# speedinghzl/DSRG

Hardware: AMD Instinct MI355X
Metric: images/sec DSRG train step (VGG16 321x321, 21-class) (higher is better)
Workload: dtype bf16 backbone (fp32 master weights) + f32/f64 supervision path

## Files before the change

### dsrg_amd/csrc/conv_igemm.hip

```cpp
#include "common.h"
#include <algorithm>
#include <cstdlib>
#include <cstring>
#include <functional>
#include <map>
#include <mutex>
#include <queue>
#include <vector>

namespace dsrg {
namespace {
typedef __attribute__((ext_vector_type(8))) __bf16 bf16x8;
typedef __attribute__((ext_vector_type(2))) __bf16 bf16x2;
typedef __attribute__((ext_vector_type(2))) float f32x2;
typedef __attribute__((ext_vector_type(16))) float f32x16;
typedef __attribute__((ext_vector_type(4))) float f32x4;
typedef __attribute__((address_space(3))) void lds_void;

constexpr int kBM = 256, kBN = 256;
constexpr int kOutRow = 128 * 2 + 16;
constexpr int kOutWave = 64 * kOutRow;
constexpr uint32_t kOob = 0x80000000u;
constexpr int kRowTab = 8 * kOutWave;
constexpr int kRowTabBytes = kBM * 4;
// ... 354 lines not shown
            const uint4 v = *reinterpret_cast<const uint4 *>(O + p * kOutRow + ch * 16);
            if (m >= 0 && chv) *reinterpret_cast<uint4 *>(G.y + (size_t)m * a.Cout + nw + ch * 8) = v;
        }
        return;
    }
    uint4 mk[16];
    if (G.mask) {
#pragma unroll
        for (int it = 0; it < 16; it++) {
            const int m = row_pixel(wm * 64 + it * 4 + (lane >> 4));
            mk[it] = (m >= 0 && chv) ? *reinterpret_cast<const uint4 *>(G.mask + (size_t)m * a.Cout + nw + (lane & 15) * 8) : make_uint4(0, 0, 0, 0);
        }
    } else {
#pragma unroll
        for (int it = 0; it < 16; it++) mk[it] = make_uint4(0x3f803f80u, 0x3f803f80u, 0x3f803f80u, 0x3f803f80u);
    }
    float cs[8] = {0, 0, 0, 0, 0, 0, 0, 0};
#pragma unroll
    for (int it = 0; it < 16; it++) {
        const int p = it * 4 + (lane >> 4), ch = lane & 15;
        const int m = row_pixel(wm * 64 + p);
        const uint4 v = *reinterpret_cast<const uint4 *>(O + p * kOutRow + ch * 16);
        uint32_t w4[4] = {v.x, v.y, v.z, v.w};
        const uint32_t y4[4] = {mk[it].x, mk[it].y, mk[it].z, mk[it].w};
#pragma unroll
        for (int e = 0; e < 4; e++) {
            const uint32_t lo = (int16_t)(y4[e] & 0xffffu) > 0 ? 0x0000ffffu : 0u;
            const uint32_t hi = (int32_t)y4[e] >= 0x10000 ? 0xffff0000u : 0u;
            w4[e] &= lo | hi;
            cs[2 * e] += __uint_as_float(w4[e] << 16);
            cs[2 * e + 1] += __uint_as_float(w4[e] & 0xffff0000u);
        }
        if (m >= 0 && chv) *reinterpret_cast<uint4 *>(G.y + (size_t)m * a.Cout + nw + ch * 8) = make_uint4(w4[0], w4[1], w4[2], w4[3]);
    }
    if (G.colsum) {
#pragma unroll
        for (int e = 0; e < 8; e++) {
            cs[e] += __shfl_xor(cs[e], 16);
            cs[e] += __shfl_xor(cs[e], 32);
        }
        float *slab = reinterpret_cast<float *>(O);
        if (lane < 16) {
            *reinterpret_cast<float4 *>(slab + lane * 8) = make_float4(cs[0], cs[1], cs[2], cs[3]);
            *reinterpret_cast<float4 *>(slab + lane * 8 + 4) = make_float4(cs[4], cs[5], cs[6], cs[7]);
        }
        __syncthreads();
        if (wm == 0) {
            const float *s0 = reinterpret_cast<const float *>(ig_lds + (wn * 4 + 0) * kOutWave);
            const float *s1 = reinterpret_cast<const float *>(ig_lds + (wn * 4 + 1) * kOutWave);
            const float *s2 = reinterpret_cast<const float *>(ig_lds + (wn * 4 + 2) * kOutWave);
            const float *s3 = reinterpret_cast<const float *>(ig_lds + (wn * 4 + 3) * kOutWave);
            float *dst = G.colsum + (size_t)tm * a.Cout + nw;
            dst[lane] = (s0[lane] + s1[lane]) + (s2[lane] + s3[lane]);
            if (nw + lane + 64 < a.Cout) dst[lane + 64] = (s0[lane + 64] + s1[lane + 64]) + (s2[lane + 64] + s3[lane + 64]);
        }
    }
}


__global__ __launch_bounds__(512, 2) void conv_igemm_kernel_64x2(IgemmArgs a) { conv_igemm_body(a, (int)blockIdx.x, (int)gridDim.x); }

struct IgemmSkArgs {
    IgemmArgs base;
    float *ws;
    uint32_t *flags;
    int units, tiles_total;
};
constexpr int kSkParts = 4;
using f32x4v = decltype(__builtin_amdgcn_raw_buffer_load_b128(rsrc_t(), 0, 0, 0));

__global__ __launch_bounds__(512, 2) void conv_igemm_sk_kernel(IgemmSkArgs k) {
    using C = ICfg<64, 2>;
    const IgemmArgs &a = k.base;
    extern __shared__ __attribute__((aligned(16))) unsigned char ig_lds[];
    const int tid = threadIdx.x, lane = tid & 63;
    const int wv = __builtin_amdgcn_readfirstlane(tid >> 6);
    const int l15 = lane & 15, g4 = lane >> 4;
    const int wn = wv >> 2, wm = wv & 3;
    int unit;
    {
        const int total = (int)gridDim.x, id = (int)blockIdx.x;
        const int q = total >> 3, r = total & 7, xcd = id & 7, kk = id >> 3;
        unit = (xcd < r ? xcd * (q + 1) : r * (q + 1) + (xcd - r) * q) + kk;
    }
    const int taps = a.taps, Cin = a.Cin, W = a.W, H = a.H;
    const int ktot = taps * Cin;
    const int nsteps = (Cin >> 6) * taps;
    const long long total_steps = (long long)k.tiles_total * nsteps;
    auto unit_start = [&](int u) { return (long long)u * total_steps / k.units; };
    const long long g1 = unit_start(unit + 1);
    const IgemmFrag fr(lane);
    const rsrc_t rws = make_rsrc(k.ws, (size_t)k.units * 32 * 512 * 16);
    const float floor_ = a.relu ? 0.0f : -__builtin_inff();

    for (long long g = unit_start(unit); g < g1;) {
        const int tile = (int)(g / nsteps);
        const int sb = (int)(g - (long long)tile * nsteps);
        const int se = (int)min((long long)nsteps, sb + (g1 - g));
        int t = tile;
        const int grp = t / a.tiles_per_group;
        t -= grp * a.tiles_per_group;
        const int tm = t / a.tiles_n, tn = t - tm * a.tiles_n;
        const int m0 = tm * kBM, n0 = tn * kBN;
        const IgemmGroup G = a.g[grp];
        const rsrc_t rx = make_rsrc(G.x, (size_t)a.M * Cin * 2);
        const rsrc_t rw = make_rsrc(G.w, (size_t)a.Cout * ktot * 2);
        const bool active = n0 + wn * 128 < a.Cout;

        uint32_t pbase0, wbase0, pvalid01 = 0, pvalid23 = 0;
        {
            const int r0 = wv * 32 + lane / C::CPR;
            const int c0 = (lane % C::CPR) ^ C::swz(r0);
            pbase0 = (uint32_t)(m0 + r0) * (uint32_t)(Cin * 2) + (uint32_t)c0 * 16u;
            wbase0 = (uint32_t)(n0 + r0) * (uint32_t)(ktot * 2) + (uint32_t)c0 * 16u;
#pragma unroll
            for (int i = 0; i < C::IPW; i++) {
                const int m = m0 + r0 + i * C::RPI;
                uint32_t valid = 0;
                if (m < a.M) {
                    const int hw = H * W;
                    const int bimg = m / hw, rem = m - bimg * hw, y = rem / W, x = rem - y * W;
                    if (taps == 9) {
#pragma unroll
                        for (int tap = 0; tap < 9; tap++) {
                            const int yy = y + (tap / 3 - 1) * G.dil, xx = x + (tap % 3 - 1) * G.dil;
                            if (yy >= 0 && yy < H && xx >= 0 && xx < W) valid |= 1u << tap;
                        }
                    } else {
                        valid = 1u;
                    }
                }
                if (i < 2) pvalid01 |= valid << (16 * i); else pvalid23 |= valid << (16 * (i - 2));
            }
        }
        auto issue = [&](int stage, int s) {
            const int cc = s / taps, tap = s - cc * taps;
            int dy = 0, dx = 0;
            if (taps == 9) { dy = tap / 3 - 1; dx = tap - (tap / 3) * 3 - 1; }
            const int toff = (dy * G.dil * W + dx * G.dil) * Cin * 2 + cc * 128;
            unsigned char *P = ig_lds + stage * C::STAGE + wv * (32 * C::ROW);
            unsigned char *Wt = P + kBM * C::ROW;
#pragma unroll
            for (int i = 0; i < C::IPW; i++) {
                const uint32_t bits = (i < 2 ? pvalid01 : pvalid23) >> (16 * (i & 1) + tap);
                const uint32_t off = ((pbase0 + (uint32_t)(i * C::RPI * Cin * 2)) ^ ((i & 1) ? 64u : 0u)) + (uint32_t)toff;
                __builtin_amdgcn_raw_ptr_buffer_load_lds(rx, (lds_void *)(P + i * (C::RPI * C::ROW)), 16, (bits & 1u) ? off : kOob, 0, 0, 0);
            }
#pragma unroll
            for (int i = 0; i < C::IPW; i++)
                __builtin_amdgcn_raw_ptr_buffer_load_lds(rw, (lds_void *)(Wt + i * (C::RPI * C::ROW)), 16, (i & 1) ? wbase0 ^ 64u : wbase0,
                                                         (uint32_t)s * C::ROW + (uint32_t)(i * C::RPI * ktot * 2), 0, 0);
        };

        f32x4 acc[8][4];
#pragma unroll
        for (int i = 0; i < 8; i++)
#pragma unroll
            for (int j = 0; j < 4; j++)
#pragma unroll
                for (int r = 0; r < 4; r++) acc[i][j][r] = 0.0f;

        issue(0, sb);
        if (!active) {
            for (int s = sb; s < se; s++) {
                wait_vm_barrier<0>();
                if (s + 1 < se) issue(((s - sb) & 1) ^ 1, s + 1);
            }
        } else {
            for (int s = sb; s < se; s++) {
                const int stage = (s - sb) & 1;
                wait_vm_barrier<0>();
                const bool more = s + 1 < se, late = wv >= 4;
                if (more && !late) issue(stage ^ 1, s + 1);
                igemm_mma_step(ig_lds + stage * C::STAGE + wm * (64 * C::ROW), ig_lds + stage * C::STAGE + kBM * C::ROW + wn * (128 * C::ROW), fr, acc,
                               more && late, [&]() { issue(stage ^ 1, s + 1); });
            }
        }
        __syncthreads();

        if (sb != 0) {
            if (active) {
#pragma unroll
                for (int i = 0; i < 8; i++)
#pragma unroll
                    for (int j = 0; j < 4; j++) {
                        f32x4v v = {__float_as_uint(acc[i][j][0]), __float_as_uint(acc[i][j][1]), __float_as_uint(acc[i][j][2]), __float_as_uint(acc[i][j][3])};
                        __builtin_amdgcn_raw_buffer_store_b128(v, rws, (uint32_t)((i * 4 + j) * 512 + tid) * 16u,
                                                               (uint32_t)unit * (32u * 512u * 16u), 16);
                    }
            }
            asm volatile("s_waitcnt vmcnt(0)" ::: "memory");
            __syncthreads();
            if (tid == 0) __hip_atomic_store(k.flags + unit, 1u, __ATOMIC_RELAXED, __HIP_MEMORY_SCOPE_AGENT);
        } else {
            bool ok = true;
            int nparts = 0;
            if (se != nsteps) {
                const long long tile_end = (long long)(tile + 1) * nsteps;
                while (unit + 1 + nparts < k.units && unit_start(unit + 1 + nparts) < tile_end) nparts++;
                volatile int &sk_ok = *reinterpret_cast<volatile int *>(ig_lds);
                if (tid == 0) {
                    int good = nparts <= kSkParts ? 1 : 0;
                    for (int p = 0; p < nparts && good; p++) {
                        unsigned spins = 0;
                        while (__hip_atomic_load(k.flags + unit + 1 + p, __ATOMIC_RELAXED, __HIP_MEMORY_SCOPE_AGENT) != 1u) {
                            __builtin_amdgcn_s_sleep(8);
                            if (++spins > (1u << 24)) { good = 0; break; }
                        }
                    }
                    if (good) __builtin_amdgcn_fence(__ATOMIC_ACQUIRE, "agent");
                    else __hip_atomic_store(k.flags + k.units, 1u, __ATOMIC_RELAXED, __HIP_MEMORY_SCOPE_AGENT);
                    sk_ok = good;
                }
                __syncthreads();
                ok = sk_ok != 0;
                __syncthreads();
            }
            if (active) {
                const float poison = ok ? 0.0f : __builtin_nanf("");
                unsigned char *O = ig_lds + wv * kOutWave;
                const int nw = n0 + wn * 128;
                const rsrc_t rb = make_rsrc(G.bias, G.bias ? (size_t)a.Cout * 4 : 0);
                const uint32_t seed_g = a.seed_lo + (uint32_t)grp * 0x9E3779B9u;
                f32x4v shares[2][kSkParts];
                float bq[2][4];
                auto fetch = [&](int gi, f32x4v (&dst)[kSkParts], float (&bias4)[4]) {
                    const int i = gi >> 2;
                    const uint32_t off = (uint32_t)(gi * 512 + tid) * 16u;
#pragma unroll
                    for (int p = 0; p < kSkParts; p++)
                        dst[p] = __builtin_amdgcn_raw_buffer_load_b128(rws, p < nparts ? off : kOob, (uint32_t)(unit + 1 + p) * (32u * 512u * 16u), 0);
#pragma unroll
                    for (int e = 0; e < 4; e++) bias4[e] = ld_f32(rb, (uint32_t)(nw + i * 16 + g4 * 4 + e) * 4u);
                };
                fetch(0, shares[0], bq[0]);
#pragma unroll
                for (int gi = 0; gi < 32; gi++) {
                    const int i = gi >> 2, j = gi & 3;
                    if (gi + 1 < 32) fetch(gi + 1, shares[(gi + 1) & 1], bq[(gi + 1) & 1]);
                    __builtin_amdgcn_sched_barrier(0);
                    const int nl = i * 16 + g4 * 4;
                    float s0 = acc[i][j][0], s1 = acc[i][j][1], s2 = acc[i][j][2], s3 = acc[i][j][3];
#pragma unroll
                    for (int p = 0; p < kSkParts; p++) {
                        const f32x4v pv = shares[gi & 1][p];
                        s0 += __uint_as_float(pv[0]); s1 += __uint_as_float(pv[1]); s2 += __uint_as_float(pv[2]); s3 += __uint_as_float(pv[3]);
                    }
                    float v0 = s0 + bq[gi & 1][0], v1 = s1 + bq[gi & 1][1], v2 = s2 + bq[gi & 1][2], v3 = s3 + bq[gi & 1][3];
                    v0 = fmaxf(v0, floor_) + poison; v1 = fmaxf(v1, floor_) + poison; v2 = fmaxf(v2, floor_) + poison; v3 = fmaxf(v3, floor_) + poison;
                    if (a.drop_thresh) {
                        const uint32_t m = (uint32_t)(m0 + wm * 64 + j * 16 + l15);
                        const uint32_t h = dropout_bytes((m * (uint32_t)a.Cout + (uint32_t)(nw + nl)) >> 2, seed_g, a.seed_hi);
                        v0 = (h & 0xffu) >= a.drop_thresh ? v0 * a.drop_scale : 0.0f;
                        v1 = ((h >> 8) & 0xffu) >= a.drop_thresh ? v1 * a.drop_scale : 0.0f;
                        v2 = ((h >> 16) & 0xffu) >= a.drop_thresh ? v2 * a.drop_scale : 0.0f;
                        v3 = (h >> 24) >= a.drop_thresh ? v3 * a.drop_scale : 0.0f;
                    }
                    *reinterpret_cast<uint2 *>(O + (j * 16 + l15) * kOutRow + nl * 2) = make_uint2(pack2(v0, v1), pack2(v2, v3));
                    __builtin_amdgcn_sched_barrier(0);
                }
#pragma unroll 4
                for (int it = 0; it < 16; it++) {
                    const int p = it * 4 + (lane >> 4), ch = lane & 15;
                    const int m = m0 + wm * 64 + p;
                    const uint4 v = *reinterpret_cast<const uint4 *>(O + p * kOutRow + ch * 16);
                    if (m < a.M) *reinterpret_cast<uint4 *>(G.y + (size_t)m * a.Cout + nw + ch * 8) = v;
                }
            }
        }
        g += se - sb;
        __syncthreads();
    }
}

struct WgradGroup {
    const uint16_t *x;
    const uint16_t *g;
    float *part;
    int dil, pad_;
};
struct IgemmWgradArgs {
    WgradGroup g[4];
    int ngroups, B, H, W, Cin, Cout, taps, M, tiles_n, tiles_c, ksplit, kchunk, tiles_per_group;
    int stagger;
    int compact;
    int xcd_mix;
    int skip_rows;
    int nent;
    const uint32_t *plan;
};
constexpr int kPlanHdr = 2 * 4 * 9;
constexpr int kWRow = 512;
constexpr int kWTile = 64 * kWRow;
constexpr int kWStage = 2 * kWTile;
typedef __attribute__((__vector_size__(4 * sizeof(__bf16)))) __bf16 bf16x4v;
typedef __attribute__((address_space(3))) unsigned char lds_u8;

__device__ __forceinline__ bf16x8 tr_frag8(lds_u8 *p) {
    bf16x4v lo = __builtin_amdgcn_ds_read_tr16_b64_v4bf16(reinterpret_cast<__attribute__((address_space(3))) bf16x4v *>(p));
    bf16x4v hi = __builtin_amdgcn_ds_read_tr16_b64_v4bf16(reinterpret_cast<__attribute__((address_space(3))) bf16x4v *>(p + 4 * kWRow));
    return __builtin_shufflevector(lo, hi, 0, 1, 2, 3, 4, 5, 6, 7);
}

__device__ __forceinline__ void conv_igemm_wgrad_body(const IgemmWgradArgs &a, const int bid, const int nblk) {
    extern __shared__ __attribute__((aligned(16))) unsigned char ig_lds[];
    const int tid = threadIdx.x, lane = tid & 63;
    const int wv = __builtin_amdgcn_readfirstlane(tid >> 6);
    const int l31 = lane & 31, kgrp = lane >> 5, i16 = lane & 15, gq = lane >> 4;
    const int wn = wv >> 2, wm = wv & 3;

    const int tiles = a.tiles_n * a.tiles_c;
    int grp, split, t, ksp = a.ksplit;
    size_t plane = 0;
    if (a.plan) {
        const int ncb_ = (a.Cin + 255) >> 8, tpe = a.tiles_n * ncb_;
        const int xcd = bid & 7, k = bid >> 3, pos = k / tpe, te = k - pos * tpe, e = pos * 8 + xcd;
        if (e >= a.nent) return;
        const uint32_t w = a.plan[kPlanHdr + e];
        grp = (int)(w & 3u);
        const int ptap = (int)((w >> 2) & 15u), tn_ = te / ncb_;
        split = (int)((w >> 6) & 255u);
        ksp = (int)((w >> 14) & 255u);
        t = tn_ * a.tiles_c + ptap * ncb_ + (te - tn_ * ncb_);
        plane = (size_t)a.plan[2 * (grp * 9 + ptap) + 1] + (size_t)split;
    } else if (a.xcd_mix) {
        const int id = bid, xcd = id & 7, k = id >> 3;
        if (a.ksplit >= 8) {
            const int per_group = (a.ksplit >> 3) * tiles;
            grp = k / per_group;
            const int r = k - grp * per_group, sl = r / tiles;
            t = r - sl * tiles;
            split = xcd + 8 * sl;
        } else {
            const int xpc = 8 / a.ksplit, sub = xcd % xpc, per_group = tiles / xpc;
            split = xcd / xpc;
            grp = k / per_group;
            t = sub + xpc * (k - grp * per_group);
        }
    } else {
        const int total = nblk, id = bid;
        const int q = total >> 3, r = total & 7, xcd = id & 7, k = id >> 3;
        t = (xcd < r ? xcd * (q + 1) : r * (q + 1) + (xcd - r) * q) + k;
        grp = t / a.tiles_per_group;
        t -= grp * a.tiles_per_group;
        split = t / tiles;
        t -= split * tiles;
    }
    const int tn = t / a.tiles_c, tc = t - tn * a.tiles_c;
    const WgradGroup G = a.g[grp];
    const int taps = a.taps, Cin = a.Cin, Cout = a.Cout, W = a.W, H = a.H;
    const bool two = Cin == 128 && taps == 9;
    const int ncb = two ? 1 : (Cin + 255) >> 8;
    const int tap = two ? 2 * tc : tc / ncb, c0 = two ? 0 : (tc - tap * ncb) << 8, n0 = tn << 8;
    const int tdy = (taps == 9 && !two) ? (tap / 3 - 1) * G.dil : 0, tdx = (taps == 9 && !two) ? (tap % 3 - 1) * G.dil : 0;
    const bool compact = a.compact && !two && taps == 9;
    const int ry0 = compact ? max(0, -tdy) : 0, rx0 = compact ? max(0, -tdx) : 0;
    const int rh_ = compact ? H - abs(tdy) : H, rw_ = compact ? W - abs(tdx) : W;
    const int rh = max(rh_, 1), rw = max(rw_, 1);
    const int area = rh * rw;
    const int Kc = (rh_ > 0 && rw_ > 0) ? a.B * area : 0;
    const int kchunk = compact ? (((Kc + ksp - 1) / ksp + 63) >> 6) << 6 : a.kchunk;
    const int mbeg = split * kchunk, mend = min(Kc, mbeg + kchunk);
    const int nsteps = mend > mbeg ? (mend - mbeg + 63) >> 6 : 0;

    const rsrc_t rx = make_rsrc(G.x, (size_t)a.M * Cin * 2);
    const rsrc_t rg = make_rsrc(G.g, (size_t)a.M * Cout * 2);

    int pm[4], pb[4], py[4], px[4], ldy[4], ldx[4], ltapoff[4];
    uint32_t srcoff[4], xsrcoff[4];
    bool ltap[4];
#pragma unroll
    for (int i = 0; i < 4; i++) {
        const int r = wv * 8 + i * 2 + (lane >> 5);
        const int q = lane & 31, p = (q >> 2) ^ (r & 3);
        srcoff[i] = (uint32_t)(p * 64 + (q & 3) * 16);
        const int mytap = two ? tap + (p >> 2) : tap;
        xsrcoff[i] = two ? (uint32_t)((p & 3) * 64 + (q & 3) * 16) : srcoff[i];
        if (!two && (uint32_t)(c0 * 2) + xsrcoff[i] >= (uint32_t)(Cin * 2)) xsrcoff[i] |= 0x80000000u;
        if ((uint32_t)(n0 * 2) + srcoff[i] >= (uint32_t)(Cout * 2)) srcoff[i] |= 0x80000000u;
        ltap[i] = mytap < taps;
        ldy[i] = taps == 9 ? (mytap / 3 - 1) * G.dil : 0;
        ldx[i] = taps == 9 ? (mytap % 3 - 1) * G.dil : 0;
        ltapoff[i] = (ldy[i] * W + ldx[i]) * Cin * 2 + c0 * 2;
        const int m = mbeg + r;
        pm[i] = m;
        const int mm = m < Kc ? m : 0;
        pb[i] = mm / area;
        const int rem = mm - pb[i] * area;
        py[i] = rem / rw;
        px[i] = rem - py[i] * rw;
    }
    const int qW = 64 / rw, rW = 64 - qW * rw;

    auto advance = [&]() {
#pragma unroll
        for (int i = 0; i < 4; i++) {
            pm[i] += 64;
            px[i] += rW;
            py[i] += qW;
            if (px[i] >= rw) { px[i] -= rw; py[i] += 1; }
            while (py[i] >= rh) { py[i] -= rh; pb[i] += 1; }
        }
    };
    auto issue = [&](int stage) {
        unsigned char *A = ig_lds + stage * kWStage + wv * (8 * kWRow);
        unsigned char *Bt = A + kWTile;
        int pix[4];
#pragma unroll
        for (int i = 0; i < 4; i++) pix[i] = compact ? (pb[i] * H + ry0 + py[i]) * W + rx0 + px[i] : pm[i];
#pragma unroll
        for (int i = 0; i < 4; i++) {
            const bool live = pm[i] < mend;
            const uint32_t vo = live ? (uint32_t)pix[i] * (uint32_t)(Cout * 2) + (uint32_t)(n0 * 2) + srcoff[i] : kOob;
            __builtin_amdgcn_raw_ptr_buffer_load_lds(rg, (lds_void *)(A + i * (2 * kWRow)), 16, vo, 0, 0, 0);
        }
#pragma unroll
        for (int i = 0; i < 4; i++) {
            const int yy = ry0 + py[i] + ldy[i], xx = rx0 + px[i] + ldx[i];
            const bool live = ltap[i] && pm[i] < mend && yy >= 0 && yy < H && xx >= 0 && xx < W;
            const uint32_t vo = live ? (uint32_t)(pix[i] * (Cin * 2) + ltapoff[i]) + xsrcoff[i] : kOob;
            __builtin_amdgcn_raw_ptr_buffer_load_lds(rx, (lds_void *)(Bt + i * (2 * kWRow)), 16, vo, 0, 0, 0);
        }
        advance();
    };

    f32x16 acc[4][2];
#pragma unroll
    for (int i = 0; i < 4; i++)
#pragma unroll
        for (int j = 0; j < 2; j++)
#pragma unroll
            for (int r = 0; r < 16; r++) acc[i][j][r] = 0.0f;

    const int swz = (i16 >> 2) & 3;
    const uint32_t lane_off = (uint32_t)((kgrp * 8 + (i16 >> 2)) * kWRow + (gq & 1) * 32 + (i16 & 3) * 8);
    uint32_t aoff[4], boff[2];
#pragma unroll
    for (int i = 0; i < 4; i++) aoff[i] = lane_off + (uint32_t)(((wn * 4 + i) ^ swz) * 64);
#pragma unroll
    for (int j = 0; j < 2; j++) boff[j] = lane_off + (uint32_t)(kWTile + ((wm * 2 + j) ^ swz) * 64);
    lds_u8 *lds = (lds_u8 *)ig_lds;

    const bool may_skip = a.skip_rows && !compact && abs(tdy) * W >= 64 && tdy > -H && tdy < H;
    const int hw_ = H * W;
    auto step_dead = [&](int st) -> bool {
        const int p0 = mbeg + st * 64, p1 = min(p0 + 63, mend - 1);
        const int b0 = p0 / hw_, b1 = p1 / hw_;
        if (b0 != b1) return false;
        const int y0 = (p0 - b0 * hw_) / W, y1 = (p1 - b0 * hw_) / W;
        return y1 + tdy < 0 || y0 + tdy >= H;
    };
    int cur = 0;
    auto seek = [&]() {
        if (may_skip)
            while (cur < nsteps && step_dead(cur)) { advance(); cur++; }
    };
    seek();
    bool have = cur < nsteps;
    if (have) { issue(0); cur++; }
    for (int s = 0; have; s++) {
        wait_vm_barrier<0>();
        seek();
        const bool more = cur < nsteps, late = a.stagger && wv >= 4;
        if (more && !late) { issue((s + 1) & 1); cur++; }
        lds_u8 *st = lds + (s & 1) * kWStage;
        bf16x8 af[2][4], bfr[2][2];
#pragma unroll
        for (int i = 0; i < 4; i++) af[0][i] = tr_frag8(st + aoff[i]);
#pragma unroll
        for (int j = 0; j < 2; j++) bfr[0][j] = tr_frag8(st + boff[j]);
#pragma unroll
        for (int ks = 0; ks < 4; ks++) {
            if (ks + 1 < 4) {
#pragma unroll
                for (int i = 0; i < 4; i++) af[(ks + 1) & 1][i] = tr_frag8(st + (ks + 1) * (16 * kWRow) + aoff[i]);
#pragma unroll
                for (int j = 0; j < 2; j++) bfr[(ks + 1) & 1][j] = tr_frag8(st + (ks + 1) * (16 * kWRow) + boff[j]);
            }
            __builtin_amdgcn_sched_barrier(0);
#pragma unroll
            for (int i = 0; i < 4; i++)
#pragma unroll
                for (int j = 0; j < 2; j++)
                    acc[i][j] = __builtin_amdgcn_mfma_f32_32x32x16_bf16(af[ks & 1][i], bfr[ks & 1][j], acc[i][j], 0, 0, 0);
            __builtin_amdgcn_sched_barrier(0);
            if (ks == 0 && more && late) { issue((s + 1) & 1); cur++; }
        }
        have = more;
    }
    float *pp = a.plan ? G.part + plane * ((size_t)Cout * Cin) : G.part + (size_t)split * ((size_t)Cout * taps * Cin);
    const size_t prow = a.plan ? (size_t)Cin : (size_t)taps * Cin;
#pragma unroll
    for (int i = 0; i < 4; i++)
#pragma unroll
        for (int j = 0; j < 2; j++) {
            const int col = wm * 64 + j * 32 + l31;
            const int etap = two ? tap + (col >> 7) : tap, c = two ? (col & 127) : c0 + col;
            if (etap < taps && c < Cin && n0 + wn * 128 + i * 32 < Cout) {
#pragma unroll
                for (int r = 0; r < 16; r++) {
                    const int n = n0 + wn * 128 + i * 32 + (r & 3) + 8 * (r >> 2) + 4 * kgrp;
                    pp[(size_t)n * prow + (a.plan ? 0 : etap * Cin) + c] = acc[i][j][r];
                }
            }
        }
}

__global__ __launch_bounds__(512, 2) void conv_igemm_wgrad_kernel(IgemmWgradArgs a) { conv_igemm_wgrad_body(a, (int)blockIdx.x, (int)gridDim.x); }

struct IgemmBwdArgs {
    IgemmArgs d;
    IgemmWgradArgs w;
    int nd, nd_pad, nw;
    int w_first, nw_pad;
};
__global__ __launch_bounds__(512, 2) void conv_igemm_bwd_kernel(IgemmBwdArgs a) {
    const int id = (int)blockIdx.x;
    if (a.w_first) {
        if (id < a.nw_pad) {
            if (id < a.nw) conv_igemm_wgrad_body(a.w, id, a.nw);
        } else if (id - a.nw_pad < a.nd) {
            conv_igemm_body(a.d, id - a.nw_pad, a.nd);
        }
        return;
    }
    if (id < a.nd_pad) {
        if (id < a.nd) conv_igemm_body(a.d, id, a.nd);
    } else {
        conv_igemm_wgrad_body(a.w, id - a.nd_pad, a.nw);
    }
}

struct WgradReduceArgs {
    const float *part[4];
    void *gw[4];
    int ksplit;
    int cin4;
    const uint32_t *plan;
    size_t plane4;
    size_t n4;
    const float *scale;
    size_t per_o4;
};
template <bool BF16_OUT>
__global__ __launch_bounds__(256) void conv_igemm_wgrad_reduce_kernel(WgradReduceArgs a) {
    const size_t e = (size_t)blockIdx.x * 256 + threadIdx.x;
    if (e >= a.n4) return;
    const float4 *p = reinterpret_cast<const float4 *>(a.part[blockIdx.y]) + e;
    void *gw = a.gw[blockIdx.y];
    int ksplit = a.ksplit;
    size_t stride = a.n4;
    if (a.plan) {
        const size_t n = e / a.per_o4, rem = e - n * a.per_o4;
        const int tap = (int)(rem / (size_t)a.cin4), c4 = (int)(rem - (size_t)tap * a.cin4);
        const uint32_t *row = a.plan + 2 * ((int)blockIdx.y * 9 + tap);
        ksplit = (int)row[0];
        stride = a.plane4;
        p = reinterpret_cast<const float4 *>(a.part[0]) + (size_t)row[1] * a.plane4 + n * (size_t)a.cin4 + c4;
    }
    float4 s = ksplit > 0 ? p[0] : make_float4(0.0f, 0.0f, 0.0f, 0.0f);
    int k = 1;
    for (; k + 8 <= ksplit; k += 8) {
        float4 v[8];
#pragma unroll
        for (int u = 0; u < 8; u++) v[u] = p[(size_t)(k + u) * stride];
#pragma unroll
        for (int u = 0; u < 8; u++) { s.x += v[u].x; s.y += v[u].y; s.z += v[u].z; s.w += v[u].w; }
    }
    for (; k < ksplit; k++) {
        const float4 v = p[(size_t)k * stride];
        s.x += v.x; s.y += v.y; s.z += v.z; s.w += v.w;
    }
    if (a.scale) {
        const float f = a.scale[e / a.per_o4];
        s.x *= f; s.y *= f; s.z *= f; s.w *= f;
    }
    if (BF16_OUT) reinterpret_cast<uint2 *>(gw)[e] = make_uint2(pack2(s.x, s.y), pack2(s.z, s.w));
    else reinterpret_cast<float4 *>(gw)[e] = s;
}


__global__ __launch_bounds__(256) void pack_conv_weight_kernel(const float *w, uint16_t *fwd, uint16_t *dg, int cout, int cin, int taps,
                                                               int plain, const float *scale) {
    __shared__ uint16_t tile[64][64 + 4];
    const int ob = blockIdx.x, cb = blockIdx.y, tap = blockIdx.z, t = threadIdx.x;
    const int r = t >> 4, q = t & 15;
#pragma unroll
    for (int i = 0; i < 4; i++) {
        const int o = r + 16 * i;
        const size_t src = ((size_t)(ob * 64 + o) * taps + tap) * cin + cb * 64 + q * 4;
        float4 v = *reinterpret_cast<const float4 *>(w + src);
        if (scale) {
            const float f = scale[ob * 64 + o];
            v.x *= f; v.y *= f; v.z *= f; v.w *= f;
        }
        const uint2 pk = make_uint2(pack2(v.x, v.y), pack2(v.z, v.w));
        if (fwd) *reinterpret_cast<uint2 *>(fwd + (plain ? src : (((size_t)(ob * 64 + o) * (cin >> 6) + cb) * taps + tap) * 64 + q * 4)) = pk;
        *reinterpret_cast<uint2 *>(&tile[o][q * 4]) = pk;
    }
    if (!dg) return;
    __syncthreads();
#pragma unroll
    for (int i = 0; i < 4; i++) {
        const int c = r + 16 * i;
        const uint32_t lo = (uint32_t)tile[q * 4 + 0][c] | ((uint32_t)tile[q * 4 + 1][c] << 16);
        const uint32_t hi = (uint32_t)tile[q * 4 + 2][c] | ((uint32_t)tile[q * 4 + 3][c] << 16);
        const size_t dst = plain ? ((size_t)(cb * 64 + c) * taps + (taps - 1 - tap)) * cout + ob * 64 + q * 4
                                 : (((size_t)(cb * 64 + c) * (cout >> 6) + ob) * taps + (taps - 1 - tap)) * 64 + q * 4;
        *reinterpret_cast<uint2 *>(dg + dst) = make_uint2(lo, hi);
    }
}

}

bool conv_igemm_supported(int cin, int cout, int k) {
    return (k == 1 || k == 3) && cin >= 64 && cin % 64 == 0 && cout >= 128 && cout % 128 == 0;
}
static bool conv_igemm_launchable(int cin, int cout, int k) {
    return (k == 1 || k == 3) && cin >= 64 && cin % 64 == 0 && (cout == 64 || (cout >= 128 && cout % 128 == 0));
}

std::atomic<int> g_igemm_variant{-1};
static int igemm_variant() {
    const int v = g_igemm_variant.load(std::memory_order_relaxed);
    return (v < 0 || v == 2 || v == 5) ? 3 : v;
}

static int igemm_cus() {
    static const int n = [] {
        int dev = 0, c = 0;
        if (hipGetDevice(&dev) != hipSuccess || hipDeviceGetAttribute(&c, hipDeviceAttributeMultiprocessorCount, dev) != hipSuccess || c < 8) c = 256;
        return c;
    }();
    return n;
}
size_t conv_igemm_workspace() { return (size_t)igemm_cus() * (32 * 512 * 16) + ((size_t)igemm_cus() + 1 + 63) / 64 * 256; }

struct ColsumArgs {
    const float *part[4];
    float *out[4];
    int rows, cout;
};
__global__ __launch_bounds__(1024) void igemm_colsum_kernel(ColsumArgs a) {
    __shared__ float red[16][64];
    colsum_block(a.part[blockIdx.y], a.out[blockIdx.y], a.rows, a.cout, (int)blockIdx.x, red);
}

int launch_igemm_colsum(const float *const *parts, float *const *outs, int ngroups, int rows, int cout, hipStream_t stream) {
    if (ngroups < 1 || ngroups > 4 || cout % 64 || rows < 1) return set_error(DSRG_ERR_INVALID, "column sums: 1..4 groups, 64 | channels");
    {
        int g = 0;
        while (g < ngroups && defer_reduction(0, parts[g], outs[g], rows, cout)) g++;
        if (g == ngroups) return DSRG_OK;
        if (g > 0) return set_error(DSRG_ERR_INVALID, "column sums: the deferred-reduction list filled up in the middle of a launch's groups");
    }
    ColsumArgs c;
    memset(&c, 0, sizeof(c));
    for (int g = 0; g < ngroups; g++) { c.part[g] = parts[g]; c.out[g] = outs[g]; }
    c.rows = rows; c.cout = cout;
    hipLaunchKernelGGL(igemm_colsum_kernel, dim3(cout / 64, ngroups), dim3(1024), 0, stream, c);
    DSRG_LAUNCH_CHECK();
    return DSRG_OK;
}

static bool conv_igemm_row_tiles(int H, int W) {
    if (W > kBM / 2) return false;
    const int r = kBM / W, bands = (H + r - 1) / r;
    return (long long)bands * kBM * 10 <= (long long)H * W * 11 + 10LL * kBM;
}
static size_t conv_igemm_pixel_tiles(int B, int H, int W) {
    const long long M = (long long)B * H * W;
    size_t t = (size_t)((M + kBM - 1) / kBM);
    if (W <= kBM && conv_igemm_row_tiles(H, W)) {
        const int r = kBM / W;
        const size_t tr = (size_t)B * ((H + r - 1) / r);
        if (tr > t) t = tr;
    }
    return t;
}
size_t conv_igemm_colsum_workspace(int ngroups, int B, int H, int W, int cout) {
    return (size_t)ngroups * conv_igemm_pixel_tiles(B, H, W) * (size_t)cout * sizeof(float);
}

static uint32_t tap_mask_rect(int H, int W, int d, int y0, int y1, int x0, int x1) {
    uint32_t m = 0;
    for (int tap = 0; tap < 9; tap++) {
        const int dy = (tap / 3 - 1) * d, dx = (tap % 3 - 1) * d;
        if (std::max(y0, -dy) < std::min(y1, H - dy) && std::max(x0, -dx) < std::min(x1, W - dx)) m |= 1u << tap;
    }
    return m;
}
static int axis_bands(int n, int d, int (*out)[2]) {
    if (d >= n) { out[0][0] = 0; out[0][1] = n; return 1; }
    const int lo = std::min(d, n - d), hi = std::max(d, n - d), cut[4] = {0, lo, hi, n};
    int k = 0;
    for (int i = 0; i < 3; i++)
        if (cut[i + 1] > cut[i]) { out[k][0] = cut[i]; out[k][1] = cut[i + 1]; k++; }
    return k;
}
struct HostClass { int y0, y1, x0, x1; uint32_t mask; };
static int build_classes(int H, int W, int d, HostClass *c) {
    int yb[3][2], xb[3][2];
    const int ny = axis_bands(H, d, yb), nx = axis_bands(W, d, xb);
    int n = 0;
    for (int i = 0; i < ny; i++)
        for (int j = 0; j < nx; j++) c[n++] = HostClass{yb[i][0], yb[i][1], xb[j][0], xb[j][1], tap_mask_rect(H, W, d, yb[i][0], yb[i][1], xb[j][0], xb[j][1])};
    std::stable_sort(c, c + n, [](const HostClass &a, const HostClass &b) { return __builtin_popcount(a.mask) > __builtin_popcount(b.mask); });
    return n;
}
static long long tile_taps(int B, int H, int W, int d, int mode) {
    const long long M = (long long)B * H * W;
    long long tot = 0;
    if (mode == 2) {
        HostClass c[kMaxClasses];
        const int n = build_classes(H, W, d, c);
        long long q0[kMaxClasses + 1];
        q0[0] = 0;
        for (int k = 0; k < n; k++) q0[k + 1] = q0[k] + (long long)B * (c[k].y1 - c[k].y0) * (c[k].x1 - c[k].x0);
        for (long long t0 = 0; t0 < M; t0 += kBM) {
            const long long t1 = std::min(M, t0 + kBM);
            uint32_t m = 0;
            for (int k = 0; k < n; k++)
                if (q0[k] < t1 && q0[k + 1] > t0) m |= c[k].mask;
            tot += __builtin_popcount(m);
        }
    } else if (mode == 1) {
        const int r = kBM / W;
        for (int y0 = 0; y0 < H; y0 += r) tot += (long long)B * __builtin_popcount(tap_mask_rect(H, W, d, y0, std::min(H, y0 + r), 0, W));
    } else {
        for (long long t0 = 0; t0 < M; t0 += kBM) {
            const long long t1 = std::min(M, t0 + kBM);
            uint32_t m = 0;
            for (long long p = t0; p < t1;) {
                const int rem = (int)(p % ((long long)H * W)), y = rem / W, x = rem % W;
                const int x1 = (int)std::min<long long>(W, x + (t1 - p));
                m |= tap_mask_rect(H, W, d, y, y + 1, x, x1);
                p += x1 - x;
            }
            tot += __builtin_popcount(m);
        }
    }
    return tot;
}

static thread_local IgemmArgs *t_prep_d = nullptr;
static thread_local IgemmWgradArgs *t_prep_w = nullptr;
static thread_local int *t_prep_grid = nullptr;
static thread_local int t_force_ksplit = 0;
static thread_local const float *t_wgrad_scale = nullptr;
static thread_local const void *t_res = nullptr;
static thread_local int t_split_cin = 0;

int launch_conv_igemm(const void *const *x, const void *const *w, const float *const *bias, void *const *y, const int *dil,
                      int ngroups, int B, int H, int W, int cin, int cout, int k, int relu, float drop_p, unsigned long long seed,
                      void *workspace, size_t workspace_bytes, hipStream_t stream, const void *const *mask, float out_scale,
                      float *const *colsum, void *colsum_ws, size_t colsum_ws_bytes) {
    if (ngroups < 1 || ngroups > 4) return set_error(DSRG_ERR_INVALID, "conv_igemm: 1..4 groups");
    if (colsum && (!colsum_ws || colsum_ws_bytes < conv_igemm_colsum_workspace(ngroups, B, H, W, cout)))
        return set_error(DSRG_ERR_INVALID, "conv_igemm: column-sum scratch missing or too small");
    if (!conv_igemm_launchable(cin, cout, k))
        return set_error(DSRG_ERR_UNSUPPORTED, "conv_igemm: cin %% 64 == 0, cout %% 128 == 0 (or cout = 64), k in (1, 3) required (got %d, %d, %d)",
                         cin, cout, k);
    const long long M = (long long)B * H * W;
    if (M <= 0 || M * cin * 2 >= 0x7fffffffLL || (long long)cout * k * k * cin * 2 >= 0x7fffffffLL || M * cout * 2 >= 0x7fffffff00LL)
        return set_error(DSRG_ERR_UNSUPPORTED, "conv_igemm: tensor too large for 32-bit buffer offsets");
    IgemmArgs a;
    memset(&a, 0, sizeof(a));
    for (int g = 0; g < ngroups; g++) {
        a.g[g].x = static_cast<const uint16_t *>(x[g]);
        a.g[g].w = static_cast<const uint16_t *>(w[g]);
        a.g[g].bias = bias ? bias[g] : nullptr;
        a.g[g].y = static_cast<uint16_t *>(y[g]);
        a.g[g].dil = dil ? dil[g] : 1;
        a.g[g].mask = mask ? static_cast<const uint16_t *>(mask[g]) : nullptr;
        a.g[g].colsum = colsum ? static_cast<float *>(colsum_ws) + (size_t)g * conv_igemm_pixel_tiles(B, H, W) * cout : nullptr;
        a.g[g].res = static_cast<const uint16_t *>(t_res);
        if (!a.g[g].x || !a.g[g].w || !a.g[g].y || (mask && !mask[g]) || (colsum && !colsum[g]))
            return set_error(DSRG_ERR_INVALID, "conv_igemm: null pointer");
    }
    a.out_scale = out_scale;
    a.xrow = cin * 2;
    if (t_split_cin > 0) {
        a.xrow = 3 * t_split_cin * 2;
        a.cpp = t_split_cin / 64;
        a.out_f32 = 1;
    }
    a.skip_taps = igemm_variant() != 6;
    const bool fused_bwd = mask || colsum || t_res;
    if (t_res && (colsum || ngroups != 1 || drop_p != 0.0f || t_split_cin))
        return set_error(DSRG_ERR_UNSUPPORTED, "conv_igemm: a residual goes with one group, no column sums, no dropout");
    a.ngroups = ngroups; a.B = B; a.H = H; a.W = W; a.Cin = cin; a.Cout = cout; a.taps = k * k; a.relu = relu; a.M = (int)M;
    a.tiles_m = (int)((M + kBM - 1) / kBM);
    a.tiles_n = (cout + kBN - 1) / kBN;
    a.tiles_per_group = a.tiles_m * a.tiles_n;
    if (drop_p < 0.0f || drop_p >= 1.0f) return set_error(DSRG_ERR_INVALID, "conv_igemm: 0 <= dropout probability < 1");
    a.drop_thresh = (uint32_t)(drop_p * 256.0f + 0.5f);
    if (a.drop_thresh > 255) a.drop_thresh = 255;
    a.drop_scale = 256.0f / (float)(256 - (int)a.drop_thresh);
    a.seed_lo = (uint32_t)seed; a.seed_hi = (uint32_t)(seed >> 32);
    static LdsGrant grant[2];
    a.stagger = igemm_variant() >= 3;
    const bool default_form = igemm_variant() == 3 || igemm_variant() == 8 || igemm_variant() == 9;
    const dim3 block(512);
    const int units = igemm_cus(), tiles_total = a.tiles_per_group * ngroups, nsteps = (cin / 64) * k * k;
    const bool sk_wins = tiles_total * 100 <= units * 60, sk_forced = igemm_variant() == 4;
    if (!fused_bwd && t_split_cin == 0 && cout % 128 == 0 && workspace && workspace_bytes >= conv_igemm_workspace() && ((default_form && sk_wins) || sk_forced) &&
        (long long)tiles_total * nsteps >= (long long)units * 8 && tiles_total * 3 >= units) {
        IgemmSkArgs sk;
// ... 509 lines not shown
```

Baseline: 2011.

## Switch wgrad inner loop to 16x16x32 MFMA with ring-buffered LDS fragment reads

Rewrites the weight-gradient igemm inner loop to use 16x16x32 bf16 MFMAs over 8x4 accumulator tiles instead of 32x32x16 over 4x2. It changes the LDS swizzle and source-offset layout to match, and reads fragments through a small prefetch ring. The epilogue now writes four contiguous floats per lane as a vector store, replacing sixteen scalar strided stores. The aim is to overlap LDS transposed reads with MFMAs and to coalesce the partial-sum writes, at the risk of different register pressure and a different MFMA issue rate.

```diff
diff --git a/dsrg_amd/csrc/conv_igemm.hip b/dsrg_amd/csrc/conv_igemm.hip
--- a/dsrg_amd/csrc/conv_igemm.hip
+++ b/dsrg_amd/csrc/conv_igemm.hip
@@ -680,11 +680,34 @@
     return __builtin_shufflevector(lo, hi, 0, 1, 2, 3, 4, 5, 6, 7);
 }
 
+template <class LateIssue>
+__device__ __forceinline__ void wgrad_mma_step(lds_u8 *st, const uint32_t (&aoff)[8], const uint32_t (&boff)[4], f32x4 (&acc)[8][4],
+                                               const bool late, LateIssue &&late_issue) {
+    constexpr int RING = kAhead + 1;
+    bf16x8 xq[2][4], gr[RING];
+    auto read_g = [&](int u) { return tr_frag8(st + (u >> 3) * (32 * kWRow) + aoff[u & 7]); };
+#pragma unroll
+    for (int j = 0; j < 4; j++) xq[0][j] = tr_frag8(st + boff[j]);
+#pragma unroll
+    for (int u = 0; u < kAhead; u++) gr[u] = read_g(u);
+#pragma unroll
+    for (int u = 0; u < 16; u++) {
+        if (u + kAhead < 16) gr[(u + kAhead) % RING] = read_g(u + kAhead);
+        if (u < 4) xq[1][u] = tr_frag8(st + 32 * kWRow + boff[u]);
+        __builtin_amdgcn_sched_barrier(0);
+#pragma unroll
+        for (int j = 0; j < 4; j++)
+            acc[u & 7][j] = __builtin_amdgcn_mfma_f32_16x16x32_bf16(xq[u >> 3][j], gr[u % RING], acc[u & 7][j], 0, 0, 0);
+        __builtin_amdgcn_sched_barrier(0);
+        if (u == 3 && late) late_issue();
+    }
+}
+
 __device__ __forceinline__ void conv_igemm_wgrad_body(const IgemmWgradArgs &a, const int bid, const int nblk) {
     extern __shared__ __attribute__((aligned(16))) unsigned char ig_lds[];
     const int tid = threadIdx.x, lane = tid & 63;
     const int wv = __builtin_amdgcn_readfirstlane(tid >> 6);
-    const int l31 = lane & 31, kgrp = lane >> 5, i16 = lane & 15, gq = lane >> 4;
+    const int i16 = lane & 15, gq = lane >> 4;
     const int wn = wv >> 2, wm = wv & 3;
 
     const int tiles = a.tiles_n * a.tiles_c;
@@ -750,10 +773,11 @@
 #pragma unroll
     for (int i = 0; i < 4; i++) {
         const int r = wv * 8 + i * 2 + (lane >> 5);
-        const int q = lane & 31, p = (q >> 2) ^ (r & 3);
-        srcoff[i] = (uint32_t)(p * 64 + (q & 3) * 16);
-        const int mytap = two ? tap + (p >> 2) : tap;
-        xsrcoff[i] = two ? (uint32_t)((p & 3) * 64 + (q & 3) * 16) : srcoff[i];
+        const int q = lane & 31;
+        const int u = (q >> 1) ^ ((r & 3) | (((r >> 3) & 1) << 2));
+        srcoff[i] = (uint32_t)(u * 32 + (q & 1) * 16);
+        const int mytap = two ? tap + (u >> 3) : tap;
+        xsrcoff[i] = two ? (uint32_t)((u & 7) * 32 + (q & 1) * 16) : srcoff[i];
         if (!two && (uint32_t)(c0 * 2) + xsrcoff[i] >= (uint32_t)(Cin * 2)) xsrcoff[i] |= 0x80000000u;
         if ((uint32_t)(n0 * 2) + srcoff[i] >= (uint32_t)(Cout * 2)) srcoff[i] |= 0x80000000u;
         ltap[i] = mytap < taps;
@@ -802,21 +826,21 @@
         advance();
     };
 
-    f32x16 acc[4][2];
-#pragma unroll
-    for (int i = 0; i < 4; i++)
-#pragma unroll
-        for (int j = 0; j < 2; j++)
-#pragma unroll
-            for (int r = 0; r < 16; r++) acc[i][j][r] = 0.0f;
-
-    const int swz = (i16 >> 2) & 3;
-    const uint32_t lane_off = (uint32_t)((kgrp * 8 + (i16 >> 2)) * kWRow + (gq & 1) * 32 + (i16 & 3) * 8);
-    uint32_t aoff[4], boff[2];
-#pragma unroll
-    for (int i = 0; i < 4; i++) aoff[i] = lane_off + (uint32_t)(((wn * 4 + i) ^ swz) * 64);
-#pragma unroll
-    for (int j = 0; j < 2; j++) boff[j] = lane_off + (uint32_t)(kWTile + ((wm * 2 + j) ^ swz) * 64);
+    f32x4 acc[8][4];
+#pragma unroll
+    for (int i = 0; i < 8; i++)
+#pragma unroll
+        for (int j = 0; j < 4; j++)
+#pragma unroll
+            for (int r = 0; r < 4; r++) acc[i][j][r] = 0.0f;
+
+    const int swz = (i16 >> 2) | ((gq & 1) << 2);
+    const uint32_t lane_off = (uint32_t)((gq * 8 + (i16 >> 2)) * kWRow + (i16 & 3) * 8);
+    uint32_t aoff[8], boff[4];
+#pragma unroll
+    for (int i = 0; i < 8; i++) aoff[i] = lane_off + (uint32_t)(((wn * 8 + i) ^ swz) * 32);
+#pragma unroll
+    for (int j = 0; j < 4; j++) boff[j] = lane_off + (uint32_t)(kWTile + ((wm * 4 + j) ^ swz) * 32);
     lds_u8 *lds = (lds_u8 *)ig_lds;
 
     const bool may_skip = a.skip_rows && !compact && abs(tdy) * W >= 64 && tdy > -H && tdy < H;
@@ -836,52 +860,28 @@
     seek();
     bool have = cur < nsteps;
     if (have) { issue(0); cur++; }
+    const bool late = a.stagger && wv >= 4;
     for (int s = 0; have; s++) {
         wait_vm_barrier<0>();
         seek();
-        const bool more = cur < nsteps, late = a.stagger && wv >= 4;
+        const bool more = cur < nsteps;
         if (more && !late) { issue((s + 1) & 1); cur++; }
-        lds_u8 *st = lds + (s & 1) * kWStage;
-        bf16x8 af[2][4], bfr[2][2];
-#pragma unroll
-        for (int i = 0; i < 4; i++) af[0][i] = tr_frag8(st + aoff[i]);
-#pragma unroll
-        for (int j = 0; j < 2; j++) bfr[0][j] = tr_frag8(st + boff[j]);
-#pragma unroll
-        for (int ks = 0; ks < 4; ks++) {
-            if (ks + 1 < 4) {
-#pragma unroll
-                for (int i = 0; i < 4; i++) af[(ks + 1) & 1][i] = tr_frag8(st + (ks + 1) * (16 * kWRow) + aoff[i]);
-#pragma unroll
-                for (int j = 0; j < 2; j++) bfr[(ks + 1) & 1][j] = tr_frag8(st + (ks + 1) * (16 * kWRow) + boff[j]);
-            }
-            __builtin_amdgcn_sched_barrier(0);
-#pragma unroll
-            for (int i = 0; i < 4; i++)
-#pragma unroll
-                for (int j = 0; j < 2; j++)
-                    acc[i][j] = __builtin_amdgcn_mfma_f32_32x32x16_bf16(af[ks & 1][i], bfr[ks & 1][j], acc[i][j], 0, 0, 0);
-            __builtin_amdgcn_sched_barrier(0);
-            if (ks == 0 && more && late) { issue((s + 1) & 1); cur++; }
-        }
+        wgrad_mma_step(lds + (s & 1) * kWStage, aoff, boff, acc, more && late, [&]() { issue((s + 1) & 1); cur++; });
         have = more;
     }
     float *pp = a.plan ? G.part + plane * ((size_t)Cout * Cin) : G.part + (size_t)split * ((size_t)Cout * taps * Cin);
     const size_t prow = a.plan ? (size_t)Cin : (size_t)taps * Cin;
 #pragma unroll
-    for (int i = 0; i < 4; i++)
-#pragma unroll
-        for (int j = 0; j < 2; j++) {
-            const int col = wm * 64 + j * 32 + l31;
+    for (int i = 0; i < 8; i++) {
+        const int n = n0 + wn * 128 + i * 16 + i16;
+#pragma unroll
+        for (int j = 0; j < 4; j++) {
+            const int col = wm * 64 + j * 16 + 4 * gq;
             const int etap = two ? tap + (col >> 7) : tap, c = two ? (col & 127) : c0 + col;
-            if (etap < taps && c < Cin && n0 + wn * 128 + i * 32 < Cout) {
-#pragma unroll
-                for (int r = 0; r < 16; r++) {
-                    const int n = n0 + wn * 128 + i * 32 + (r & 3) + 8 * (r >> 2) + 4 * kgrp;
-                    pp[(size_t)n * prow + (a.plan ? 0 : etap * Cin) + c] = acc[i][j][r];
-                }
-            }
-        }
+            if (etap < taps && c < Cin && n0 + wn * 128 + i * 16 < Cout)
+                *reinterpret_cast<f32x4 *>(pp + (size_t)n * prow + (a.plan ? 0 : etap * Cin) + c) = acc[i][j];
+        }
+    }
 }
 
 __global__ __launch_bounds__(512, 2) void conv_igemm_wgrad_kernel(IgemmWgradArgs a) { conv_igemm_wgrad_body(a, (int)blockIdx.x, (int)gridDim.x); }
```

New measurement: 2015 (median of 3 runs). No clear change (+0.2%).
